# marict/nnue-vision

Measured on AMD Instinct MI355X. Metric: NNUE training images/sec (full step: fwd+bwd+clip+SGD), higher is better.
Workload: dtype f32; 1 GPU; c2: NNUE 32x32 grid 10x10x8 F=800 -> 1024/128/32 -> 10, batch 512/GPU, SGD m0.9 wd2e-4 clip1.0; global_batch=512, parallelism=dp1, launch=hipGraph, steps_per_graph=26, max_active_features=453

## Files before the change

### nnue-vision_amd/csrc/classifier_kernels.hip

```cpp
#include <type_traits>
#include <cstdlib>
#include <cstring>

#include "common.h"
#include "small_wgrad.h"

namespace {

using f32x4 = __attribute__((ext_vector_type(4))) float;

__device__ __forceinline__ float act_fn(float z, float clip) {
  const float r = z <= 0.0f ? 0.0f : z;
  return (clip > 0.0f && r > clip) ? clip : r;
}
__device__ __forceinline__ float gate_fn(float d, float h, float clip) {
  if (clip > 0.0f) return (h > 0.0f && h < clip) ? d : 0.0f;
  return h <= 0.0f ? 0.0f : d;
}

__device__ __forceinline__ float l0_at(const float* __restrict__ xr, int k, int half, int pairwise) {
  if (!pairwise) return xr[k];
  return k < half ? xr[k] * xr[k + half] : xr[k - half];
}

// ... 621 lines not shown
    }
  }
  const float b2v = (VEC && og < L3) ? b2[og] : 0.0f, b3v = (VEC && og < C) ? b3[og] : 0.0f;
  const int64_t y = labels[b];
  for (int j = tid; j < L2; j += NT) {
    float z = b1[j];
    int s = 0;
    for (; s + 8 <= ksplit; s += 8) {
      float v[8];
#pragma unroll
      for (int u = 0; u < 8; ++u) v[u] = part[((size_t)(s + u) * B + b) * L2 + j];
#pragma unroll
      for (int u = 0; u < 8; ++u) z += v[u];
    }
    for (; s < ksplit; ++s) z += part[((size_t)s * B + b) * L2 + j];
    const float h = act_fn(z, clip);
    h1s[j] = h;
    h1[(size_t)b * L2 + j] = h;
  }
  __syncthreads();
  for (int j0 = 0; j0 < L3; j0 += NT / 4) {
    const int j = j0 + og;
    float z = 0.f;
    if (j < L3) {
      const float* __restrict__ wr = w2 + (size_t)j * L2;
      if constexpr (VEC) {
        int k = 4 * part4;
        if (j0 == 0) {
#pragma unroll
          for (int i = 0; i < kPre2; ++i) {
            const int kk = 4 * (part4 + 4 * i);
            if (kk < L2) z = tail_dot4(w2v[i], *reinterpret_cast<const float4*>(h1s + kk), z);
          }
          k += 16 * kPre2;
        }
        for (; k < L2; k += 16) z = tail_dot4(*reinterpret_cast<const float4*>(wr + k), *reinterpret_cast<const float4*>(h1s + k), z);
      } else {
        for (int k = part4; k < L2; k += 4) z = fmaf(wr[k], h1s[k], z);
      }
    }
    z += __shfl_xor(z, 1);
    z += __shfl_xor(z, 2);
    if (j < L3 && part4 == 0) {
      const float h = act_fn(z + ((VEC && j0 == 0) ? b2v : b2[j]), clip);
      h2s[j] = h;
      h2[(size_t)b * L3 + j] = h;
    }
  }
  __syncthreads();
  for (int c0 = 0; c0 < C; c0 += NT / 4) {
    const int c = c0 + og;
    float z = 0.f;
    if (c < C) {
      const float* __restrict__ wr = w3 + (size_t)c * L3;
      if constexpr (VEC) {
        int k = 4 * part4;
        if (c0 == 0) {
#pragma unroll
          for (int i = 0; i < kPre3; ++i) {
            const int kk = 4 * (part4 + 4 * i);
            if (kk < L3) z = tail_dot4(w3v[i], *reinterpret_cast<const float4*>(h2s + kk), z);
          }
          k += 16 * kPre3;
        }
        for (; k < L3; k += 16) z = tail_dot4(*reinterpret_cast<const float4*>(wr + k), *reinterpret_cast<const float4*>(h2s + k), z);
      } else {
        for (int k = part4; k < L3; k += 4) z = fmaf(wr[k], h2s[k], z);
      }
    }
    z += __shfl_xor(z, 1);
    z += __shfl_xor(z, 2);
    if (c < C && part4 == 0) {
      z += (VEC && c0 == 0) ? b3v : b3[c];
      lgs[c] = z;
      logits[(size_t)b * C + c] = z;
    }
  }
  __syncthreads();
  float mx = -INFINITY, se = 0.f;
  if (C <= 64) {
    const int lane = tid & 63;
    const float v[1] = {lane < C ? lgs[lane] : -INFINITY};
    float m1[1], s1[1];
    ce_wave_stats<1>(v, lane < C, m1, s1);
    mx = m1[0];
    se = s1[0];
  } else {
    for (int c = tid; c < C; c += NT) mx = fmaxf(mx, lgs[c]);
    mx = block_reduce_nt<NT>(mx, true, red);
    for (int c = tid; c < C; c += NT) se += expf(lgs[c] - mx);
    se = block_reduce_nt<NT>(se, false, red);
  }
  const bool ok = y >= 0 && y < C;
  if (tid == 0) sample_loss[b] = ok ? nnue_ce_sample_loss(mx, lgs[y], se) : 0.0f;
  const float inv = 1.0f / se;
  __syncthreads();
  for (int c = tid; c < C; c += NT) {
    const float g = ok ? ce_dlogit(lgs[c], mx, inv, c == y, scale_over_b) : 0.0f;
    lgs[c] = g;
    d_logits[(size_t)b * C + c] = g;
  }
  __syncthreads();
  for (int j0 = 0; j0 < L3; j0 += 32) {
    const int j = j0 + (tid & 31), cp = tid >> 5;
    part_s[cp][tid & 31] = j < L3 ? dz2_slice<S>(lgs, w3 + j, cp, C, L3) : 0.0f;
    __syncthreads();
    if (cp == 0 && j < L3) {
      float q[S];
#pragma unroll
      for (int i = 0; i < S; ++i) q[i] = part_s[i][tid];
      const float v = gate_fn(slice_tree<S>(q), h2s[j], clip);
      dz2s[j] = v;
      d_z2[(size_t)b * L3 + j] = v;
    }
    __syncthreads();
  }
  for (int k = tid; k < L2; k += NT) {
    float s = 0.f;
    int j = 0;
    for (; j + 16 <= L3; j += 16) {
      float w[16];
#pragma unroll
      for (int u = 0; u < 16; ++u) w[u] = w2[(size_t)(j + u) * L2 + k];
#pragma unroll
      for (int u = 0; u < 16; ++u) s = fmaf(dz2s[j + u], w[u], s);
    }
    for (; j < L3; ++j) s = fmaf(dz2s[j], w2[(size_t)j * L2 + k], s);
    const float v = gate_fn(s, h1s[k], clip);
    d_z1[(size_t)b * L2 + k] = v;
    if (d_z1_g) d_z1_g[(size_t)g * L2 + k] = v;
  }
  __syncthreads();
}

constexpr int kTdxRows = 16, kTdxThreads = 512, kTdxMaxC = 64;

#ifdef NNUE_ABLATIONS
constexpr int kTdxClocks = 10;
struct TdxAbl { long long* clocks; };
#define NNUE_TDX_ABL_PARAM , TdxAbl abl
#define NNUE_TDX_CLOCK(i) do { if (abl.clocks && threadIdx.x == 0) abl.clocks[(size_t)blockIdx.x * kTdxClocks + (i)] = clock64(); } while (0)
#else
#define NNUE_TDX_ABL_PARAM
#define NNUE_TDX_CLOCK(i) do { } while (0)
#endif

struct TailFrags {
  float w2f[8];
  float w2b[8];
  float w3f[8];
  float b3v;
};

template <int L2, int L3>
__device__ __forceinline__ void tail_load_frags(TailFrags& f, const float* __restrict__ w2, const float* __restrict__ w3,
                                                const float* __restrict__ b3, int C, int wave, int r, int q) {
  static_assert(L2 == 128 && L3 == 32, "tail_load_frags: the wave roles are laid out for 128 / 32");
  const int t = wave & 1, kq = wave >> 1, kh = (wave >> 1) & 1;
  const bool lg = wave < 4;
#pragma unroll
  for (int i = 0; i < 8; ++i) {
    const int k = 16 * (i >> 2) + 4 * q + (i & 3);
    f.w2f[i] = w2[(16 * t + r) * L2 + 32 * kq + k];
    f.w2b[i] = w2[k * L2 + 16 * wave + r];
    const int cls = lg ? 16 * wave + r : 32 * kh + k, unit = lg ? k : 16 * t + r;
    f.w3f[i] = w3[min(cls, C - 1) * L3 + unit];
  }
  f.b3v = b3[min(16 * (wave & 3) + r, C - 1)];
}

__device__ __forceinline__ f32x4 tail_mma4(const float4& a, float b0, float b1, float b2, float b3, f32x4 acc) {
  acc = __builtin_amdgcn_mfma_f32_16x16x4f32(a.x, b0, acc, 0, 0, 0);
  acc = __builtin_amdgcn_mfma_f32_16x16x4f32(a.y, b1, acc, 0, 0, 0);
  acc = __builtin_amdgcn_mfma_f32_16x16x4f32(a.z, b2, acc, 0, 0, 0);
  acc = __builtin_amdgcn_mfma_f32_16x16x4f32(a.w, b3, acc, 0, 0, 0);
  return acc;
}

template <int L2, int L3, bool DX, bool SKIP = false>
__global__ __launch_bounds__(kTdxThreads) void tail_dx_train_kernel(
    const float* __restrict__ part, int ksplit, const float* __restrict__ b1, const float* __restrict__ w2,
    const float* __restrict__ b2, const float* __restrict__ w3, const float* __restrict__ b3, float clip,
    const int64_t* __restrict__ labels, float scale_over_b, int B, int C, float* __restrict__ h1, float* __restrict__ h2,
    float* __restrict__ logits, float* __restrict__ sample_loss, float* __restrict__ d_logits, float* __restrict__ d_z1,
    float* __restrict__ d_z2, const float* __restrict__ x, const float* __restrict__ w1, int L1, float* __restrict__ d_x,
    int m_tiles, int n_cg NNUE_TDX_ABL_PARAM) {
  constexpr int T = kTdxRows, NT = kTdxThreads, NWAVE = NT / 64;
  constexpr int NI = T * L2 / 4 / NT;
  constexpr int NCH = L2 / (16 * kBwxKC);
  static_assert(NI >= 1 && NI * NT * 4 == T * L2 && T * L3 == NT && NWAVE == 8 && T == 16,
                "tail_dx_train_kernel: unsupported layer widths");
  __shared__ __attribute__((aligned(16))) float h1s[T][L2 + 4];
  __shared__ __attribute__((aligned(16))) float dz1s[T][L2 + 4];
  __shared__ __attribute__((aligned(16))) float h2s[T][L3 + 4];
  __shared__ __attribute__((aligned(16))) float dz2s[T][L3 + 4];
  __shared__ float ps[T][4][L3];
  __shared__ __attribute__((aligned(16))) float lgs[T][kTdxMaxC + 4];
  __shared__ int64_t ys[T];
  __shared__ f32x4 xch[DX ? NWAVE : 1][64];

  const int blk = blockIdx.x, slot = blk >> 3;
  const int mt = (slot / n_cg) * 8 + (blk & 7), cg = slot % n_cg;
  if (mt >= m_tiles) return;
  const bool writer = cg == 0;
  const int row0 = mt * T;
  const int tid = threadIdx.x;
  constexpr bool skip = SKIP;
  NNUE_TDX_CLOCK(0);

  const int wave = __builtin_amdgcn_readfirstlane(tid >> 6);
  const int lane = tid & 63;
  const int r = lane & 15, q = lane >> 4;
  const int half = L1 / 2;
  const int hi = wave & 1;
  const int c0 = (cg * (NWAVE / 2) + (wave >> 1)) * 16, c1 = c0 + half, cm = hi ? c1 : c0;
  int orows[4];
#pragma unroll
  for (int e = 0; e < 4; ++e) orows[e] = row0 + 4 * q + e;
  float bw[NCH][kBwxKC][4];
  float xv[4];
  if constexpr (DX) {
#pragma unroll
    for (int n = 0; n < NCH; ++n) bwx_load_b_tile(bw[n], w1, n * 16 * kBwxKC, L1, L2, cm, r, q);
#pragma unroll
    for (int e = 0; e < 4; ++e) xv[e] = x[(size_t)min(orows[e], B - 1) * L1 + (hi ? c0 : c1) + r];
  }

  TailFrags fr;
  tail_load_frags<L2, L3>(fr, w2, w3, b3, C, wave, r, q);
  const float b2v = b2[tid % L3];
  const int64_t yv = labels[min(row0 + (tid % T), B - 1)];
  int srow[NI], scol[NI];
  float4 z4[NI];
  const float* prow[NI];
#pragma unroll
  for (int i = 0; i < NI; ++i) {
    const int f = tid + NT * i;
    srow[i] = f / (L2 / 4);
    scol[i] = 4 * (f % (L2 / 4));
    prow[i] = part + (size_t)min(row0 + srow[i], B - 1) * L2 + scol[i];
    z4[i] = make_float4(b1[scol[i]], b1[scol[i] + 1], b1[scol[i] + 2], b1[scol[i] + 3]);
  }
  const size_t slab = (size_t)B * L2;
  auto load_batch = [&](int s0, float4 (&v)[NI][16]) {
#pragma unroll
    for (int i = 0; i < NI; ++i)
#pragma unroll
      for (int u = 0; u < 16; ++u) v[i][u] = *reinterpret_cast<const float4*>(prow[i] + (size_t)min(s0 + u, ksplit - 1) * slab);
  };
  auto sum_batch = [&](int s0, const float4 (&v)[NI][16]) {
#pragma unroll
    for (int i = 0; i < NI; ++i)
#pragma unroll
      for (int u = 0; u < 16; ++u) {
        const bool add = s0 + u < ksplit;
        z4[i].x = add ? z4[i].x + v[i][u].x : z4[i].x;
        z4[i].y = add ? z4[i].y + v[i][u].y : z4[i].y;
        z4[i].z = add ? z4[i].z + v[i][u].z : z4[i].z;
        z4[i].w = add ? z4[i].w + v[i][u].w : z4[i].w;
      }
  };
  {
    float4 v[NI][16];
    load_batch(0, v);
    if (tid < T) ys[tid] = row0 + tid < B ? yv : -1;
    sum_batch(0, v);
  }
  for (int s0 = 16; s0 < ksplit; s0 += 16) {
    float4 v[NI][16];
    load_batch(s0, v);
    sum_batch(s0, v);
  }

#pragma unroll
  for (int i = 0; i < NI; ++i) {
    float4 h;
    h.x = act_fn(z4[i].x, clip); h.y = act_fn(z4[i].y, clip); h.z = act_fn(z4[i].z, clip); h.w = act_fn(z4[i].w, clip);
    *reinterpret_cast<float4*>(&h1s[srow[i]][scol[i]]) = h;
    if (writer && row0 + srow[i] < B) *reinterpret_cast<float4*>(h1 + (size_t)(row0 + srow[i]) * L2 + scol[i]) = h;
  }
  __syncthreads();
  NNUE_TDX_CLOCK(1);

  const f32x4 zero4 = (f32x4){0.f, 0.f, 0.f, 0.f};
  const int orow_t = tid / L3, ounit = tid % L3;
  {
    const int t = wave & 1, kq = wave >> 1;
    f32x4 acc = zero4;
    if constexpr (!skip) {
#pragma unroll
      for (int g = 0; g < 2; ++g) {
        const float4 a = *reinterpret_cast<const float4*>(&h1s[r][32 * kq + 16 * g + 4 * q]);
        acc = tail_mma4(a, fr.w2f[4 * g], fr.w2f[4 * g + 1], fr.w2f[4 * g + 2], fr.w2f[4 * g + 3], acc);
      }
    }
#pragma unroll
    for (int e = 0; e < 4; ++e) ps[4 * q + e][kq][16 * t + r] = acc[e];
  }
  __syncthreads();
  NNUE_TDX_CLOCK(2);
  {
    float z = ps[orow_t][0][ounit];
    z += ps[orow_t][1][ounit];
    z += ps[orow_t][2][ounit];
    z += ps[orow_t][3][ounit];
    const float h = act_fn(z + b2v, clip);
    h2s[orow_t][ounit] = h;
    if (writer && row0 + orow_t < B) h2[(size_t)(row0 + orow_t) * L3 + ounit] = h;
  }
  __syncthreads();
  NNUE_TDX_CLOCK(3);
  if (16 * wave < C) {
    const int n = 16 * wave + r;
    const bool n_in = n < C;
    f32x4 acc = zero4;
    if constexpr (!skip) {
#pragma unroll
      for (int g = 0; g < 2; ++g) {
        const float4 a = *reinterpret_cast<const float4*>(&h2s[r][16 * g + 4 * q]);
        acc = tail_mma4(a, n_in ? fr.w3f[4 * g] : 0.f, n_in ? fr.w3f[4 * g + 1] : 0.f, n_in ? fr.w3f[4 * g + 2] : 0.f,
                        n_in ? fr.w3f[4 * g + 3] : 0.f, acc);
      }
    }
    if (n_in) {
#pragma unroll
      for (int e = 0; e < 4; ++e) {
        const int rr = 4 * q + e;
        const float z = acc[e] + fr.b3v;
        lgs[rr][n] = z;
        if (writer && row0 + rr < B) logits[(size_t)(row0 + rr) * C + n] = z;
      }
    }
  }
  __syncthreads();
  NNUE_TDX_CLOCK(4);
  {
    constexpr int RW = T / NWAVE;
    const bool in = lane < C;
    float v[RW], mx[RW], se[RW];
#pragma unroll
    for (int it = 0; it < RW; ++it) v[it] = in ? lgs[wave + NWAVE * it][lane] : -INFINITY;
    ce_wave_stats_fast<RW>(v, in, mx, se);
#pragma unroll
    for (int it = 0; it < RW; ++it) {
      const int rr = wave + NWAVE * it;
      const int64_t y = ys[rr];
      const bool ok = y >= 0 && y < C;
      const float zy = ok ? lgs[rr][y] : 0.f;
      if (writer && lane == 0 && row0 + rr < B) sample_loss[row0 + rr] = ok ? nnue_ce_sample_loss(mx[it], zy, se[it]) : 0.0f;
      const float inv = 1.0f / se[it];
      if (in) {
        const float g = ok ? ce_dlogit(v[it], mx[it], inv, lane == y, scale_over_b) : 0.0f;
        lgs[rr][lane] = g;
        if (writer && row0 + rr < B) d_logits[(size_t)(row0 + rr) * C + lane] = g;
      }
    }
  }
  __syncthreads();
  NNUE_TDX_CLOCK(5);
  if (wave >= 4) {
    const int t = wave & 1, kh = (wave >> 1) & 1;
    f32x4 acc = zero4;
    if constexpr (!skip) {
#pragma unroll
      for (int g = 0; g < 2; ++g) {
        const int cb = 32 * kh + 16 * g;
        if (cb < C) {
          const int c = cb + 4 * q;
          float4 a = *reinterpret_cast<const float4*>(&lgs[r][c]);
          a.x = c < C ? a.x : 0.f; a.y = c + 1 < C ? a.y : 0.f; a.z = c + 2 < C ? a.z : 0.f; a.w = c + 3 < C ? a.w : 0.f;
          acc = tail_mma4(a, c < C ? fr.w3f[4 * g] : 0.f, c + 1 < C ? fr.w3f[4 * g + 1] : 0.f, c + 2 < C ? fr.w3f[4 * g + 2] : 0.f,
                          c + 3 < C ? fr.w3f[4 * g + 3] : 0.f, acc);
        }
      }
    }
#pragma unroll
    for (int e = 0; e < 4; ++e) ps[4 * q + e][kh][16 * t + r] = acc[e];
  }
  __syncthreads();
  NNUE_TDX_CLOCK(6);
  {
    const float s = ps[orow_t][0][ounit] + ps[orow_t][1][ounit];
    const float v = gate_fn(s, h2s[orow_t][ounit], clip);
    dz2s[orow_t][ounit] = v;
    if (writer && row0 + orow_t < B) d_z2[(size_t)(row0 + orow_t) * L3 + ounit] = v;
  }
  __syncthreads();
  NNUE_TDX_CLOCK(7);
  {
    f32x4 acc = zero4;
    if constexpr (!skip) {
#pragma unroll
      for (int g = 0; g < 2; ++g) {
        const float4 a = *reinterpret_cast<const float4*>(&dz2s[r][16 * g + 4 * q]);
        acc = tail_mma4(a, fr.w2b[4 * g], fr.w2b[4 * g + 1], fr.w2b[4 * g + 2], fr.w2b[4 * g + 3], acc);
      }
    }
    const int k = 16 * wave + r;
#pragma unroll
    for (int e = 0; e < 4; ++e) {
      const int rr = 4 * q + e;
      const float v = gate_fn(acc[e], h1s[rr][k], clip);
      dz1s[rr][k] = v;
      if (writer && row0 + rr < B) d_z1[(size_t)(row0 + rr) * L2 + k] = v;
    }
  }
  __syncthreads();
  NNUE_TDX_CLOCK(8);
  if constexpr (DX) {
    const bool row_ok = row0 + r < B;
    f32x4 acc = (f32x4){0.f, 0.f, 0.f, 0.f};
#pragma unroll
    for (int n = 0; n < NCH; ++n) {
      BwxChunk ch;
      bwx_load_a(ch, &dz1s[r][0], row_ok, n * 16 * kBwxKC, L2, q);
      bwx_mma_tile(ch.a, bw[n], acc);
    }
    xch[wave][lane] = acc;
    __syncthreads();
    const f32x4 other = xch[wave ^ 1][lane];
#pragma unroll
    for (int e = 0; e < 4; ++e) {
      const int orow = orows[e];
      if (orow >= B) continue;
      float* __restrict__ o = d_x + (size_t)orow * L1;
      if (hi) o[c1 + r] = other[e] * xv[e];
      else o[c0 + r] = fmaf(acc[e], xv[e], other[e]);
    }
  }
  NNUE_TDX_CLOCK(9);
}

struct ClsPlan {
  bool fwd_mfma, bww_mfma, bwx_mfma;
  int fwd_ksplit;
  int bww_ksplit, bww_klen;
};

int bucket_tiles(int B, int K) { return (B + 15) / 16 + K; }

bool tail_dx_supported(int B, int L1, int L2, int L3, int C, int K, int pairwise) {
  return B > 0 && K == 1 && pairwise && L1 > 0 && L1 % 128 == 0 && C >= 1 && C <= kTdxMaxC && L2 == 128 && L3 == 32;
}

ClsPlan make_plan(int B, int L1, int L2, int pairwise, int K = 1) {
  ClsPlan p{};
  p.fwd_mfma = (L1 % 32 == 0) && (L2 % 16 == 0);
  p.fwd_ksplit = 1;
  if (p.fwd_mfma) {
    const int tiles = (K > 1 ? bucket_tiles(B, K) : (B + 15) / 16) * ((L2 + 63) / 64);
    int ks = 1;
    while (tiles * ks < 1024 && L1 % (ks * 2 * 16) == 0 && L1 / (ks * 2) >= 64) ks *= 2;
    if (pairwise && ks == 1) ks = 2;
    static const int force_ks = [] { const char* e = getenv("NNUE_CLS_FWD_KSPLIT"); return e ? atoi(e) : 0; }();
    if (force_ks >= 2 && (force_ks & (force_ks - 1)) == 0 && L1 % (force_ks * 16) == 0 && L1 / force_ks >= 32) ks = force_ks;
    p.fwd_ksplit = ks;
  }
  p.bww_mfma = (L1 % 64 == 0) && (L2 % 32 == 0);
  p.bww_ksplit = 1;
  p.bww_klen = B;
  if (p.bww_mfma && K > 1) {
    const int tiles = (L2 / 32) * (L1 / 64);
    int ks = 1;
    while (tiles * ks < 512 && B / (ks * 2) >= 64) ks *= 2;
    p.bww_ksplit = ks;
    p.bww_klen = (((B + ks - 1) / ks) + 15) / 16 * 16;
  } else if (p.bww_mfma) {
    const int tiles = (L2 / 32) * (L1 / 64);
    int ks = 1;
    while (tiles * ks < 1024 && B / (ks * 2) >= 32) ks *= 2;
    p.bww_ksplit = ks;
    p.bww_klen = ((B + ks - 1) / ks + 3) / 4 * 4;
  }
  p.bwx_mfma = (L1 % 32 == 0) && (L2 % 16 == 0);
  return p;
}

int64_t plan_scratch_floats(const ClsPlan& p, int B, int L1, int L2, int L3, int K = 1) {
  const int64_t fwd = (int64_t)p.fwd_ksplit * B * L2;
  const int64_t bwd = (int64_t)B * L2 + (int64_t)B * L3 + (p.bww_ksplit > 1 ? (int64_t)p.bww_ksplit * K * L2 * L1 : 0);
  return (fwd > bwd ? fwd : bwd) + 64;
}

#include "bucket_group.h"

constexpr int kGroupThreads = 1024;
__global__ __launch_bounds__(kGroupThreads) void bucket_group_kernel(GroupArgs ga) {
  __shared__ int lds[kGroupLdsInts];
  bucket_group_body<kGroupThreads>(ga, lds);
}

Buckets no_buckets() { return Buckets{1, nullptr, nullptr, nullptr, nullptr, 0}; }

int buckets_from(const nnue_buckets* c, int B, Buckets* out, const char* who) {
  *out = no_buckets();
  if (!c || c->K <= 1) return NNUE_OK;
  NNUE_REQUIRE(c->K <= kMaxBuckets, NNUE_E_SHAPE, "%s: %d layer stacks (at most %d)", who, c->K, kMaxBuckets);
  NNUE_REQUIRE(c->bucket && c->rows && c->tile_bucket && c->seg, NNUE_E_ARG, "%s: null bucket pointer", who);
  NNUE_REQUIRE(c->tiles == bucket_tiles(B, c->K), NNUE_E_SHAPE, "%s: bucket grouping was made for another batch (tiles %d, expected %d)", who,
               c->tiles, bucket_tiles(B, c->K));
  *out = Buckets{c->K, c->bucket, c->rows, c->tile_bucket, c->seg, c->tiles};
  return NNUE_OK;
}

}

namespace {

int forward_impl(const float* x, int pairwise, const float* w1, const float* b1, const float* w2, const float* b2, const float* w3,
                 const float* b3, float clip, int B, int L1, int L2, int L3, int C, float* h1, float* h2, float* logits, void* scratch,
                 int64_t scratch_bytes, const Buckets& bk, nnue_stream_t stream) {
  NNUE_REQUIRE(x && w1 && b1 && w2 && b2 && w3 && b3 && h1 && h2 && logits && scratch, NNUE_E_ARG,
// ... 94 lines not shown

extern "C" int nnue_bucket_group(const int32_t* n, int B, int P, int K, int32_t* bucket, int32_t* rows, int32_t* tile_bucket,
                                 int32_t* seg, nnue_stream_t stream) {
  NNUE_REQUIRE(n && bucket && rows && tile_bucket && seg, NNUE_E_ARG, "nnue_bucket_group: null pointer");
  NNUE_REQUIRE(B > 0 && P >= 0 && K >= 1, NNUE_E_ARG, "nnue_bucket_group: B=%d P=%d K=%d out of range", B, P, K);
  NNUE_REQUIRE(K <= kMaxBuckets, NNUE_E_SHAPE, "nnue_bucket_group: %d layer stacks (at most %d)", K, kMaxBuckets);
  hipLaunchKernelGGL(bucket_group_kernel, dim3(1), dim3(kGroupThreads), 0, static_cast<hipStream_t>(stream),
                     GroupArgs{n, B, P, K, bucket, rows, tile_bucket, seg, bucket_tiles(B, K)});
  return nnue_launch_status("nnue_bucket_group");
}

extern "C" int nnue_classifier_forward(const float* x, int pairwise, const float* w1, const float* b1, const float* w2,
                                       const float* b2, const float* w3, const float* b3, float clip, int B, int L1,
                                       int L2, int L3, int C, float* h1, float* h2, float* logits, void* scratch,
                                       int64_t scratch_bytes, nnue_stream_t stream) {
  return forward_impl(x, pairwise, w1, b1, w2, b2, w3, b3, clip, B, L1, L2, L3, C, h1, h2, logits, scratch, scratch_bytes, no_buckets(),
                      stream);
}

extern "C" int nnue_classifier_forward_bucketed(const float* x, int pairwise, const float* w1, const float* b1, const float* w2,
                                                const float* b2, const float* w3, const float* b3, float clip, int B, int L1, int L2,
                                                int L3, int C, float* h1, float* h2, float* logits, void* scratch,
                                                int64_t scratch_bytes, const nnue_buckets* buckets, nnue_stream_t stream) {
  Buckets bk;
  const int rc = buckets_from(buckets, B, &bk, "nnue_classifier_forward_bucketed");
  if (rc != NNUE_OK) return rc;
  return forward_impl(x, pairwise, w1, b1, w2, b2, w3, b3, clip, B, L1, L2, L3, C, h1, h2, logits, scratch, scratch_bytes, bk, stream);
}

extern "C" int nnue_classifier_backward(const float* x, int pairwise, const float* w1, const float* w2, const float* w3,
                                        float clip, const float* h1, const float* h2, const float* d_logits, int B, int L1,
                                        int L2, int L3, int C, float* d_x, float* d_w1, float* d_b1, float* d_w2,
                                        float* d_b2, float* d_w3, float* d_b3, void* scratch, int64_t scratch_bytes,
                                        nnue_stream_t stream) {
  return backward_impl(x, pairwise, w1, w2, w3, clip, h1, h2, d_logits, B, L1, L2, L3, C, d_x, d_w1, d_b1, d_w2, d_b2, d_w3, d_b3, scratch,
                       scratch_bytes, no_buckets(), stream);
}

extern "C" int nnue_classifier_backward_bucketed(const float* x, int pairwise, const float* w1, const float* w2, const float* w3,
                                                 float clip, const float* h1, const float* h2, const float* d_logits, int B, int L1,
                                                 int L2, int L3, int C, float* d_x, float* d_w1, float* d_b1, float* d_w2, float* d_b2,
                                                 float* d_w3, float* d_b3, void* scratch, int64_t scratch_bytes,
                                                 const nnue_buckets* buckets, nnue_stream_t stream) {
  Buckets bk;
  const int rc = buckets_from(buckets, B, &bk, "nnue_classifier_backward_bucketed");
  if (rc != NNUE_OK) return rc;
  return backward_impl(x, pairwise, w1, w2, w3, clip, h1, h2, d_logits, B, L1, L2, L3, C, d_x, d_w1, d_b1, d_w2, d_b2, d_w3, d_b3, scratch,
                       scratch_bytes, bk, stream);
}

__global__ __launch_bounds__(256) void l1_backward_x_small_wgrad(const float* __restrict__ x, int pairwise, const float* __restrict__ w1,
                                                                 const float* __restrict__ d_z1, int B, int L1, int L2,
                                                                 float* __restrict__ d_x, int x_blocks, SmallWgrad a) {
  if ((int)blockIdx.x < x_blocks) l1_backward_x_body(x, pairwise, w1, d_z1, B, L1, L2, d_x, blockIdx.x, a.bk);
  else {
    __shared__ float red[1024];
    small_wgrad_body(a, (int)blockIdx.x - x_blocks, red);
  }
}

namespace {
struct TrainLayout {
  int64_t part, d_z1, d_z2, d_logits, slabs, d_z1_g, x_g, total;
};
TrainLayout train_layout(const ClsPlan& p, int B, int L1, int L2, int L3, int C, int K = 1) {
  TrainLayout t{};
  int64_t off = 0;
  auto take = [&](int64_t n) { const int64_t o = off; off += nnue_round_up(n, 4); return o; };
  const int64_t ext = (L1 % 64 == 0) ? L1 / 64 : 0;
  t.part = take((p.fwd_ksplit > ext ? (int64_t)p.fwd_ksplit : ext) * B * L2);
  t.d_z1 = take((int64_t)B * L2);
  t.d_z2 = take((int64_t)B * L3);
  t.d_logits = take((int64_t)B * C);
  t.slabs = take(p.bww_ksplit > 1 ? (int64_t)p.bww_ksplit * K * L2 * L1 : 0);
  const int64_t grows = K > 1 ? (int64_t)bucket_tiles(B, K) * 16 : 0;
  t.d_z1_g = take(grows * L2);
  t.x_g = take(grows * L1);
  t.total = off + 4;
  return t;
}

#ifdef NNUE_ABLATIONS
long long* g_tdx_clocks = nullptr;
int g_tdx_clock_blocks = 0;
#endif

int train_step_impl(const float* x, int pairwise, const float* w1, const float* b1, const float* w2, const float* b2, const float* w3,
                    const float* b3, float clip, const int64_t* labels, float grad_scale, int B, int L1, int L2, int L3, int C, float* h1,
                    float* h2, float* logits, float* sample_loss, float* loss, float* d_x, float* d_w1, float* d_b1, float* d_w2,
                    float* d_b2, float* d_w3, float* d_b3, void* scratch, int64_t scratch_bytes, int phases, const Buckets& bk,
                    nnue_stream_t stream) {
  NNUE_REQUIRE(x && w1 && b1 && w2 && b2 && w3 && b3 && labels && h1 && h2 && logits && sample_loss && loss && scratch,
               NNUE_E_ARG, "nnue_classifier_train_step: null pointer");
  const bool fuse_tail = phases == 123;
  if (fuse_tail) phases = 59;
  NNUE_REQUIRE(phases >= 1 && phases <= 63 && (phases & 3) && (phases & 20) != 20 && (!(phases & 32) || (phases & 19) == 19), NNUE_E_ARG,
               "nnue_classifier_train_step: phases = 1 (activations + d_x) | 2 (weight gradients + loss) [| 4: first-layer weight product beside "
               "d_x] [| 8: layer-1 slabs already at the start of scratch] [| 16 (not with 4): d_w1 comes from nnue_ftm_backward] [| 32 (with 1, 2 "
               "and 16): the small gradients and the mean loss ride in nnue_ftm_backward's launch as well] [| 64 (only as 123 = 59 + 64): the "
               "per-sample tail runs in the d_x launch]");
  const bool ext_dw1 = (phases & 16) != 0;
  const bool ext_small = (phases & 32) != 0;
  const bool ext_slabs = (phases & 8) != 0;
  const int K = bk.K;
  NNUE_REQUIRE(K == 1 || !ext_slabs, NNUE_E_ARG,
               "nnue_classifier_train_step: phases bit 8 (layer-1 slabs formed in the FeatureTransformer forward's epilogue) exists for one layer stack only");
  NNUE_REQUIRE(K == 1 || !ext_dw1 || (pairwise && L1 % 4 == 0), NNUE_E_SHAPE,
               "nnue_classifier_train_step: phases bit 16 with K > 1 needs the pairwise block and L1 %% 4 == 0");
  NNUE_REQUIRE(!ext_slabs || (pairwise && L1 % 64 == 0), NNUE_E_SHAPE,
               "nnue_classifier_train_step: phases bit 8 needs the pairwise block and L1 %% 64 == 0 (got L1=%d)", L1);
  NNUE_REQUIRE(d_w1 && d_b1 && d_w2 && d_b2 && d_w3 && d_b3, NNUE_E_ARG, "nnue_classifier_train_step: null gradient pointer");
  NNUE_REQUIRE(B > 0 && L1 > 0 && L2 > 0 && L3 > 0 && C > 0, NNUE_E_ARG,
               "nnue_classifier_train_step: B=%d L1=%d L2=%d L3=%d C=%d must be positive", B, L1, L2, L3, C);
  NNUE_REQUIRE(!pairwise || L1 % 2 == 0, NNUE_E_SHAPE, "nnue_classifier_train_step: pairwise needs an even L1 (got %d)", L1);
  const int64_t tail_lds = ((int64_t)L2 + 2 * L3 + C + 8) * 4;
  NNUE_REQUIRE(tail_lds <= 64 * 1024, NNUE_E_SHAPE, "nnue_classifier_train_step: L2+2*L3+C too large for the LDS tail");
  const ClsPlan p = make_plan(B, L1, L2, pairwise, K);
  const TrainLayout t = train_layout(p, B, L1, L2, L3, C, K);
  NNUE_REQUIRE(scratch_bytes >= t.total * (int64_t)sizeof(float), NNUE_E_SCRATCH,
               "nnue_classifier_train_step: scratch %lld < %lld bytes", (long long)scratch_bytes, (long long)(t.total * 4));
  NNUE_REQUIRE(nnue_aligned16(x) && nnue_aligned16(w1) && nnue_aligned16(scratch) && nnue_aligned16(d_w1) && nnue_aligned16(h1) &&
                   nnue_aligned16(h2),
               NNUE_E_ARG, "nnue_classifier_train_step: pointers must be 16-byte aligned");
  hipStream_t s = static_cast<hipStream_t>(stream);
  float* base = static_cast<float*>(scratch);
  float *part = base + t.part, *d_z1 = base + t.d_z1, *d_z2 = base + t.d_z2, *d_logits = base + t.d_logits, *slabs = base + t.slabs;
  const bool grouped = K > 1 && ext_dw1;
  float* d_z1_g = grouped ? base + t.d_z1_g : nullptr;
  float* x_g = grouped ? base + t.x_g : nullptr;
  const int tail_grid = grouped ? bk.tiles * 16 : B;
  const bool slab_pass = p.bww_mfma && p.bww_ksplit > 1;
  const int m_tiles = bk.rows ? bk.tiles : (B + 15) / 16;
  const bool early_bww = (phases & 4) && p.bwx_mfma && p.bww_mfma && d_x != nullptr;
  const int tail_slabs = ext_slabs ? L1 / 64 : p.fwd_ksplit;
  const int wgrad_blocks = small_wgrad_tiles(L2, L3, C) * K + 1;
  const long long count = (long long)K * L2 * L1;
  const int slab_blocks = slab_pass && !ext_dw1 ? (int)((count / 4 + 255) / 256) : 0;
  const SmallWgrad sw{d_logits, d_z2, d_z1, h1, h2, B, L2, L3, C, d_w3, d_b3, d_w2, d_b2, d_b1, sample_loss, loss, wgrad_blocks,
                      slabs, slab_pass && !ext_dw1 ? p.bww_ksplit : 0, count, d_w1, bk, p.bww_klen};
  const bool wgrad_rides = (phases & 3) == 3 && ext_dw1 && p.bwx_mfma && d_x != nullptr;
  NNUE_REQUIRE(!ext_small || wgrad_rides, NNUE_E_SHAPE,
               "nnue_classifier_train_step: phases bit 32 needs the d_x launch the small gradients otherwise ride in (MFMA shapes, d_x requested)");
  NNUE_REQUIRE(!fuse_tail || tail_dx_supported(B, L1, L2, L3, C, K, pairwise), NNUE_E_SHAPE,
               "nnue_classifier_train_step: phases 123 (tail inside the d_x launch) needs nnue_classifier_train_fused_tail_supported "
               "(B=%d L1=%d L2=%d L3=%d C=%d K=%d pairwise=%d)", B, L1, L2, L3, C, K, pairwise);
  NNUE_REQUIRE(!fuse_tail || (nnue_aligned16(w2) && nnue_aligned16(w3)), NNUE_E_ARG,
               "nnue_classifier_train_step: phases 123 needs 16-byte aligned w2 and w3");
  const bool tile_tail = tail_dx_supported(B, L1, L2, L3, C, K, pairwise);
  auto launch_tile_tail = [&](bool dx, int slabs_in) {
    const int n_cg = dx ? L1 / 32 / (kTdxThreads / 128) : 1;
    const int tdx_grid = (m_tiles + 7) / 8 * 8 * n_cg;
#ifdef NNUE_ABLATIONS
    static const int abl_skip = [] { const char* e = getenv("NNUE_CLS_ABL_SKIP_TAIL_PRODUCTS"); return e ? atoi(e) : 0; }();
    static const int abl_clocks = [] { const char* e = getenv("NNUE_CLS_ABL_TAIL_CLOCKS"); return e ? atoi(e) : 0; }();
    if (abl_clocks && tdx_grid > g_tdx_clock_blocks) {
      if (g_tdx_clocks) (void)hipFree(g_tdx_clocks);
      g_tdx_clocks = nullptr;
      g_tdx_clock_blocks = hipMalloc(&g_tdx_clocks, (size_t)tdx_grid * kTdxClocks * sizeof(long long)) == hipSuccess ? tdx_grid : 0;
    }
    if (abl_clocks && g_tdx_clocks) (void)hipMemsetAsync(g_tdx_clocks, 0, (size_t)g_tdx_clock_blocks * kTdxClocks * sizeof(long long), s);
    const TdxAbl abl{abl_clocks ? g_tdx_clocks : nullptr};
#define NNUE_TDX_ABL_ARG , abl
#else
    constexpr int abl_skip = 0;
#define NNUE_TDX_ABL_ARG
#endif
#define NNUE_TDX(DX, SKIP)                                                                                                                \
  hipLaunchKernelGGL((tail_dx_train_kernel<128, 32, DX, SKIP>), dim3(tdx_grid), dim3(kTdxThreads), 0, s, part, slabs_in, b1, w2, b2, w3, b3, \
                     clip, labels, grad_scale / (float)B, B, C, h1, h2, logits, sample_loss, d_logits, d_z1, d_z2, x, w1, L1, d_x, m_tiles, \
                     n_cg NNUE_TDX_ABL_ARG)
    if (abl_skip) {
#ifdef NNUE_ABLATIONS
      if (dx) NNUE_TDX(true, true); else NNUE_TDX(false, true);
#endif
    } else if (dx) NNUE_TDX(true, false);
    else NNUE_TDX(false, false);
#undef NNUE_TDX
#undef NNUE_TDX_ABL_ARG
  };
  if (fuse_tail) {
    launch_tile_tail(true, L1 / 64);
    return nnue_launch_status("nnue_classifier_train_step");
  }
  if (phases & 1) {
    if (ext_slabs) {
    } else if (p.fwd_mfma) {
      const long long waves = (long long)m_tiles * ((L2 + 63) / 64) * p.fwd_ksplit;
      hipLaunchKernelGGL(l1_forward_mfma, dim3((unsigned)((waves + 3) / 4)), dim3(256), 0, s, x, pairwise, w1, B, L1, L2, p.fwd_ksplit, part, bk);
    } else {
      const long long waves = (long long)B * L2;
      hipLaunchKernelGGL(l1_forward_simple, dim3((unsigned)((waves + 3) / 4)), dim3(256), 0, s, x, pairwise, w1, B, L1, L2, part, bk);
    }
    const bool vec = L2 % 4 == 0 && L3 % 4 == 0 && nnue_aligned16(w2) && nnue_aligned16(w3);
#define NNUE_TAIL(NT, V)                                                                                                                  \
  hipLaunchKernelGGL((tail_train_kernel<NT, V>), dim3(tail_grid), dim3(NT), (size_t)tail_lds, s, part, tail_slabs, b1, w2, b2, w3, b3, clip, \
                     labels, grad_scale / (float)B, B, L2, L3, C, h1, h2, logits, sample_loss, d_logits, d_z1, d_z2, bk, x, L1, x_g, d_z1_g)
    if (tile_tail) launch_tile_tail(false, tail_slabs);
    else if (C > 256) { if (vec) NNUE_TAIL(512, true); else NNUE_TAIL(512, false); }
    else { if (vec) NNUE_TAIL(128, true); else NNUE_TAIL(128, false); }
#undef NNUE_TAIL
    if (d_x) {
      if (p.bwx_mfma && early_bww) {
        const long long xw = (long long)m_tiles * (L1 / 32), ww = (long long)K * (L2 / 32) * (L1 / 64) * p.bww_ksplit;
        const int w_blocks = (int)((ww + 3) / 4);
        hipLaunchKernelGGL(l1_backward_xw_mfma, dim3((unsigned)(w_blocks + (xw + 3) / 4)), dim3(256), 0, s, x, pairwise, w1, d_z1, B, L1, L2,
                           d_x, w_blocks, p.bww_ksplit, p.bww_klen, slab_pass ? slabs : d_w1, bk);
      } else if (wgrad_rides) {
        const long long waves = (long long)m_tiles * (L1 / 32);
        const int x_blocks = (int)((waves + 3) / 4);
#ifdef NNUE_ABLATIONS
        static const int skip_small = [] { const char* e = getenv("NNUE_CLS_ABL_SKIP_SMALL"); return e ? atoi(e) : 0; }();
#else
        constexpr int skip_small = 0;
#endif
        hipLaunchKernelGGL(l1_backward_x_small_wgrad, dim3((unsigned)(x_blocks + ((skip_small || ext_small) ? 0 : wgrad_blocks))), dim3(256), 0, s, x, pairwise, w1,
                           (const float*)d_z1, B, L1, L2, d_x, x_blocks, sw);
      } else if (p.bwx_mfma) {
        const long long waves = (long long)m_tiles * (L1 / 32);
        hipLaunchKernelGGL(l1_backward_x_mfma, dim3((unsigned)((waves + 3) / 4)), dim3(256), 0, s, x, pairwise, w1, d_z1, B, L1, L2, d_x, bk);
      } else {
        const int cols = pairwise ? L1 / 2 : L1;
        hipLaunchKernelGGL(l1_backward_x_simple, dim3(B, (cols + 255) / 256), dim3(256), 0, s, x, pairwise, w1, d_z1, B, L1, L2, d_x, bk);
      }
    }
  }
  if (wgrad_rides) return nnue_launch_status("nnue_classifier_train_step");
  if (phases & 2) {
    if (early_bww || ext_dw1) {
    } else if (p.bww_mfma) {
      const long long waves = (long long)K * (L2 / 32) * (L1 / 64) * p.bww_ksplit;
      hipLaunchKernelGGL(l1_backward_w_mfma, dim3((unsigned)((waves + 3) / 4)), dim3(256), 0, s, x, pairwise, d_z1, B, L1, L2, p.bww_ksplit,
                         p.bww_klen, slab_pass ? slabs : d_w1, bk);
    } else {
      hipLaunchKernelGGL(l1_backward_w_simple, dim3(K * L2, (L1 + 255) / 256), dim3(256), 0, s, x, pairwise, d_z1, B, L1, L2, d_w1, bk);
    }
    hipLaunchKernelGGL(small_wgrad_kernel, dim3(wgrad_blocks + slab_blocks), dim3(256), 0, s, sw);
  }
  return nnue_launch_status("nnue_classifier_train_step");
}
}

#ifdef NNUE_ABLATIONS
extern "C" int nnue_cls_abl_tail_clocks(long long* out, int max_blocks) {
  if (!g_tdx_clocks || !out) return -1;
  const int n = g_tdx_clock_blocks < max_blocks ? g_tdx_clock_blocks : max_blocks;
  if (hipDeviceSynchronize() != hipSuccess) return -1;
  if (hipMemcpy(out, g_tdx_clocks, (size_t)n * kTdxClocks * sizeof(long long), hipMemcpyDeviceToHost) != hipSuccess) return -1;
  return n;
}
#endif

extern "C" int64_t nnue_classifier_train_scratch(int B, int L1, int L2, int L3, int C) {
  return nnue_classifier_train_scratch_bucketed(B, L1, L2, L3, C, 1);
}

extern "C" int64_t nnue_classifier_train_scratch_bucketed(int B, int L1, int L2, int L3, int C, int K) {
  if (B <= 0 || L1 <= 0 || L2 <= 0 || L3 <= 0 || C <= 0 || K <= 0) return 0;
  const int64_t a = train_layout(make_plan(B, L1, L2, 0, K), B, L1, L2, L3, C, K).total;
  const int64_t b = train_layout(make_plan(B, L1, L2, 1, K), B, L1, L2, L3, C, K).total;
  return (a > b ? a : b) * (int64_t)sizeof(float);
}

extern "C" int nnue_classifier_train_fused_tail_supported(int B, int L1, int L2, int L3, int C, int K, int pairwise) {
  return tail_dx_supported(B, L1, L2, L3, C, K, pairwise) ? 1 : 0;
}

extern "C" int64_t nnue_classifier_train_dz1_offset(int B, int L1, int L2, int L3, int C, int pairwise) {
  if (B <= 0 || L1 <= 0 || L2 <= 0 || L3 <= 0 || C <= 0) return -1;
  return train_layout(make_plan(B, L1, L2, pairwise), B, L1, L2, L3, C).d_z1 * (int64_t)sizeof(float);
}

extern "C" int64_t nnue_classifier_train_dz1_grouped_offset(int B, int L1, int L2, int L3, int C, int K) {
  if (B <= 0 || L1 <= 0 || L2 <= 0 || L3 <= 0 || C <= 0 || K <= 1 || K > kMaxBuckets) return -1;
  return train_layout(make_plan(B, L1, L2, 1, K), B, L1, L2, L3, C, K).d_z1_g * (int64_t)sizeof(float);
}

extern "C" int64_t nnue_classifier_train_x_grouped_offset(int B, int L1, int L2, int L3, int C, int K) {
  if (B <= 0 || L1 <= 0 || L2 <= 0 || L3 <= 0 || C <= 0 || K <= 1 || K > kMaxBuckets) return -1;
  return train_layout(make_plan(B, L1, L2, 1, K), B, L1, L2, L3, C, K).x_g * (int64_t)sizeof(float);
}

extern "C" int nnue_classifier_train_rider(int pairwise, int B, int L1, int L2, int L3, int C, const float* h1, const float* h2,
                                           const float* sample_loss, float* loss, float* d_b1, float* d_w2, float* d_b2, float* d_w3,
                                           float* d_b3, void* scratch, int64_t scratch_bytes, const nnue_buckets* buckets,
                                           nnue_cls_rider* out) {
  NNUE_REQUIRE(h1 && h2 && sample_loss && loss && d_b1 && d_w2 && d_b2 && d_w3 && d_b3 && scratch && out, NNUE_E_ARG,
               "nnue_classifier_train_rider: null pointer");
  NNUE_REQUIRE(B > 0 && L1 > 0 && L2 > 0 && L3 > 0 && C > 0, NNUE_E_ARG, "nnue_classifier_train_rider: sizes must be positive");
  Buckets bk;
  const int rc = buckets_from(buckets, B, &bk, "nnue_classifier_train_rider");
  if (rc != NNUE_OK) return rc;
  const ClsPlan p = make_plan(B, L1, L2, pairwise, bk.K);
  const TrainLayout t = train_layout(p, B, L1, L2, L3, C, bk.K);
  NNUE_REQUIRE(scratch_bytes >= t.total * (int64_t)sizeof(float), NNUE_E_SCRATCH, "nnue_classifier_train_rider: scratch %lld < %lld bytes",
               (long long)scratch_bytes, (long long)(t.total * 4));
  float* base = static_cast<float*>(scratch);
  const int wgrad_blocks = small_wgrad_tiles(L2, L3, C) * bk.K + 1;
  const SmallWgrad sw{base + t.d_logits, base + t.d_z2, base + t.d_z1, h1, h2, B, L2, L3, C, d_w3, d_b3, d_w2, d_b2, d_b1, sample_loss, loss,
                      wgrad_blocks, nullptr, 0, (long long)bk.K * L2 * L1, nullptr, bk, p.bww_klen};
  static_assert(sizeof(SmallWgrad) <= sizeof(nnue_cls_rider), "nnue_cls_rider is too small");
  memset(out, 0, sizeof(*out));
  memcpy(out, &sw, sizeof(sw));
  return NNUE_OK;
}

extern "C" int nnue_classifier_train_step(const float* x, int pairwise, const float* w1, const float* b1, const float* w2,
                                          const float* b2, const float* w3, const float* b3, float clip,
                                          const int64_t* labels, float grad_scale, int B, int L1, int L2, int L3, int C,
                                          float* h1, float* h2, float* logits, float* sample_loss, float* loss, float* d_x,
                                          float* d_w1, float* d_b1, float* d_w2, float* d_b2, float* d_w3, float* d_b3,
                                          void* scratch, int64_t scratch_bytes, int phases, nnue_stream_t stream) {
  return train_step_impl(x, pairwise, w1, b1, w2, b2, w3, b3, clip, labels, grad_scale, B, L1, L2, L3, C, h1, h2, logits, sample_loss, loss,
                         d_x, d_w1, d_b1, d_w2, d_b2, d_w3, d_b3, scratch, scratch_bytes, phases, no_buckets(), stream);
}

extern "C" int nnue_classifier_train_step_bucketed(const float* x, int pairwise, const float* w1, const float* b1, const float* w2,
                                                   const float* b2, const float* w3, const float* b3, float clip, const int64_t* labels,
                                                   float grad_scale, int B, int L1, int L2, int L3, int C, float* h1, float* h2,
                                                   float* logits, float* sample_loss, float* loss, float* d_x, float* d_w1, float* d_b1,
                                                   float* d_w2, float* d_b2, float* d_w3, float* d_b3, void* scratch,
                                                   int64_t scratch_bytes, int phases, const nnue_buckets* buckets, nnue_stream_t stream) {
  Buckets bk;
  const int rc = buckets_from(buckets, B, &bk, "nnue_classifier_train_step_bucketed");
  if (rc != NNUE_OK) return rc;
  return train_step_impl(x, pairwise, w1, b1, w2, b2, w3, b3, clip, labels, grad_scale, B, L1, L2, L3, C, h1, h2, logits, sample_loss, loss,
                         d_x, d_w1, d_b1, d_w2, d_b2, d_w3, d_b3, scratch, scratch_bytes, phases, bk, stream);
}
```

Baseline: 8.326 million images/sec.

## Defer tail kernel operand loads to just before each phase that uses them

```diff
diff --git a/nnue-vision_amd/csrc/classifier_kernels.hip b/nnue-vision_amd/csrc/classifier_kernels.hip
--- a/nnue-vision_amd/csrc/classifier_kernels.hip
+++ b/nnue-vision_amd/csrc/classifier_kernels.hip
@@ -797,21 +797,43 @@
   float b3v;
 };
 
-template <int L2, int L3>
-__device__ __forceinline__ void tail_load_frags(TailFrags& f, const float* __restrict__ w2, const float* __restrict__ w3,
-                                                const float* __restrict__ b3, int C, int wave, int r, int q) {
-  static_assert(L2 == 128 && L3 == 32, "tail_load_frags: the wave roles are laid out for 128 / 32");
-  const int t = wave & 1, kq = wave >> 1, kh = (wave >> 1) & 1;
-  const bool lg = wave < 4;
-#pragma unroll
-  for (int i = 0; i < 8; ++i) {
-    const int k = 16 * (i >> 2) + 4 * q + (i & 3);
-    f.w2f[i] = w2[(16 * t + r) * L2 + 32 * kq + k];
-    f.w2b[i] = w2[k * L2 + 16 * wave + r];
-    const int cls = lg ? 16 * wave + r : 32 * kh + k, unit = lg ? k : 16 * t + r;
-    f.w3f[i] = w3[min(cls, C - 1) * L3 + unit];
-  }
-  f.b3v = b3[min(16 * (wave & 3) + r, C - 1)];
+template <bool VEC>
+__device__ __forceinline__ void tail_load4(float* __restrict__ out, const float* __restrict__ p) {
+  if constexpr (VEC) {
+    const f32x4 v = *reinterpret_cast<const f32x4*>(p);
+#pragma unroll
+    for (int e = 0; e < 4; ++e) out[e] = v[e];
+  } else {
+#pragma unroll
+    for (int e = 0; e < 4; ++e) out[e] = p[e];
+  }
+}
+
+template <int L2, bool VEC>
+__device__ __forceinline__ void tail_load_frag_h2(TailFrags& f, const float* __restrict__ w2, int wave, int r, int q) {
+  const int t = wave & 1, kq = wave >> 1;
+#pragma unroll
+  for (int g = 0; g < 2; ++g) tail_load4<VEC>(&f.w2f[4 * g], w2 + (16 * t + r) * L2 + 32 * kq + 16 * g + 4 * q);
+}
+
+template <int L3, bool VEC>
+__device__ __forceinline__ void tail_load_frag_logits(TailFrags& f, const float* __restrict__ w3, int C, int wave, int r, int q) {
+  const int cls = min(16 * wave + r, C - 1);
+#pragma unroll
+  for (int g = 0; g < 2; ++g) tail_load4<VEC>(&f.w3f[4 * g], w3 + cls * L3 + 16 * g + 4 * q);
+}
+
+template <int L3>
+__device__ __forceinline__ void tail_load_frag_dz2(TailFrags& f, const float* __restrict__ w3, int C, int wave, int r, int q) {
+  const int t = wave & 1, kh = (wave >> 1) & 1;
+#pragma unroll
+  for (int i = 0; i < 8; ++i) f.w3f[i] = w3[min(32 * kh + 16 * (i >> 2) + 4 * q + (i & 3), C - 1) * L3 + 16 * t + r];
+}
+
+template <int L2>
+__device__ __forceinline__ void tail_load_frag_dz1(TailFrags& f, const float* __restrict__ w2, int wave, int r, int q) {
+#pragma unroll
+  for (int i = 0; i < 8; ++i) f.w2b[i] = w2[(16 * (i >> 2) + 4 * q + (i & 3)) * L2 + 16 * wave + r];
 }
 
 __device__ __forceinline__ f32x4 tail_mma4(const float4& a, float b0, float b1, float b2, float b3, f32x4 acc) {
@@ -822,7 +844,7 @@
   return acc;
 }
 
-template <int L2, int L3, bool DX, bool SKIP = false>
+template <int L2, int L3, bool DX, bool SKIP = false, bool NOLOAD = false>
 __global__ __launch_bounds__(kTdxThreads) void tail_dx_train_kernel(
     const float* __restrict__ part, int ksplit, const float* __restrict__ b1, const float* __restrict__ w2,
     const float* __restrict__ b2, const float* __restrict__ w3, const float* __restrict__ b3, float clip,
@@ -833,7 +855,7 @@
   constexpr int T = kTdxRows, NT = kTdxThreads, NWAVE = NT / 64;
   constexpr int NI = T * L2 / 4 / NT;
   constexpr int NCH = L2 / (16 * kBwxKC);
-  static_assert(NI >= 1 && NI * NT * 4 == T * L2 && T * L3 == NT && NWAVE == 8 && T == 16,
+  static_assert(L2 == 128 && L3 == 32 && NI >= 1 && NI * NT * 4 == T * L2 && T * L3 == NT && NWAVE == 8 && T == 16,
                 "tail_dx_train_kernel: unsupported layer widths");
   __shared__ __attribute__((aligned(16))) float h1s[T][L2 + 4];
   __shared__ __attribute__((aligned(16))) float dz1s[T][L2 + 4];
@@ -856,24 +878,6 @@
   const int wave = __builtin_amdgcn_readfirstlane(tid >> 6);
   const int lane = tid & 63;
   const int r = lane & 15, q = lane >> 4;
-  const int half = L1 / 2;
-  const int hi = wave & 1;
-  const int c0 = (cg * (NWAVE / 2) + (wave >> 1)) * 16, c1 = c0 + half, cm = hi ? c1 : c0;
-  int orows[4];
-#pragma unroll
-  for (int e = 0; e < 4; ++e) orows[e] = row0 + 4 * q + e;
-  float bw[NCH][kBwxKC][4];
-  float xv[4];
-  if constexpr (DX) {
-#pragma unroll
-    for (int n = 0; n < NCH; ++n) bwx_load_b_tile(bw[n], w1, n * 16 * kBwxKC, L1, L2, cm, r, q);
-#pragma unroll
-    for (int e = 0; e < 4; ++e) xv[e] = x[(size_t)min(orows[e], B - 1) * L1 + (hi ? c0 : c1) + r];
-  }
-
-  TailFrags fr;
-  tail_load_frags<L2, L3>(fr, w2, w3, b3, C, wave, r, q);
-  const float b2v = b2[tid % L3];
   const int64_t yv = labels[min(row0 + (tid % T), B - 1)];
   int srow[NI], scol[NI];
   float4 z4[NI];
@@ -886,6 +890,7 @@
     prow[i] = part + (size_t)min(row0 + srow[i], B - 1) * L2 + scol[i];
     z4[i] = make_float4(b1[scol[i]], b1[scol[i] + 1], b1[scol[i] + 2], b1[scol[i] + 3]);
   }
+  __builtin_amdgcn_sched_barrier(0);
   const size_t slab = (size_t)B * L2;
   auto load_batch = [&](int s0, float4 (&v)[NI][16]) {
 #pragma unroll
@@ -905,17 +910,31 @@
         z4[i].w = add ? z4[i].w + v[i][u].w : z4[i].w;
       }
   };
-  {
-    float4 v[NI][16];
-    load_batch(0, v);
-    if (tid < T) ys[tid] = row0 + tid < B ? yv : -1;
-    sum_batch(0, v);
-  }
+  float4 v0[NI][16];
+  load_batch(0, v0);
+  __builtin_amdgcn_sched_barrier(0);
+
+  TailFrags fr;
+  if constexpr (NOLOAD) {
+#pragma unroll
+    for (int i = 0; i < 8; ++i) fr.w2f[i] = fr.w2b[i] = fr.w3f[i] = 0.5f;
+    fr.b3v = 0.5f;
+  } else {
+    tail_load_frag_h2<L2, DX>(fr, w2, wave, r, q);
+    fr.b3v = b3[min(16 * (wave & 3) + r, C - 1)];
+  }
+  const float b2v = b2[tid % L3];
+  __builtin_amdgcn_sched_barrier(0);
+
+
+  ys[tid % T] = row0 + (tid % T) < B ? yv : -1;
+  sum_batch(0, v0);
   for (int s0 = 16; s0 < ksplit; s0 += 16) {
     float4 v[NI][16];
     load_batch(s0, v);
     sum_batch(s0, v);
   }
+
 
 #pragma unroll
   for (int i = 0; i < NI; ++i) {
@@ -926,6 +945,50 @@
   }
   __syncthreads();
   NNUE_TDX_CLOCK(1);
+  __builtin_amdgcn_sched_barrier(0);
+  if constexpr (!NOLOAD) tail_load_frag_logits<L3, DX>(fr, w3, C, wave & 3, r, q);
+  __builtin_amdgcn_sched_barrier(0);
+
+  const int half = L1 / 2;
+  const int hi = wave & 1;
+  const int c0 = (cg * (NWAVE / 2) + (wave >> 1)) * 16, c1 = c0 + half, cm = hi ? c1 : c0;
+  int orows[4];
+#pragma unroll
+  for (int e = 0; e < 4; ++e) orows[e] = row0 + 4 * q + e;
+  float bw[NCH][kBwxKC][4];
+  float xv[4];
+  if constexpr (DX && NOLOAD) {
+#pragma unroll
+    for (int n = 0; n < NCH; ++n)
+#pragma unroll
+      for (int u = 0; u < kBwxKC; ++u)
+#pragma unroll
+        for (int e = 0; e < 4; ++e) bw[n][u][e] = 0.5f;
+#pragma unroll
+    for (int e = 0; e < 4; ++e) xv[e] = 0.5f;
+  }
+  auto load_bw = [&](int n, int u) {
+    if constexpr (DX && !NOLOAD) {
+      const float* __restrict__ wk = w1 + (size_t)(n * 16 * kBwxKC + 16 * u + 4 * q) * L1 + r;
+#pragma unroll
+      for (int e = 0; e < 4; ++e) bw[n][u][e] = wk[(size_t)e * L1 + cm];
+    }
+  };
+  auto load_xv = [&]() {
+    if constexpr (DX && !NOLOAD) {
+#pragma unroll
+      for (int e = 0; e < 4; ++e) xv[e] = x[(size_t)min(orows[e], B - 1) * L1 + (hi ? c0 : c1) + r];
+    }
+  };
+  static_assert(NCH == 2 && NCH * 16 * kBwxKC == L2, "tail_dx_train_kernel: the W1 slice is requested in two halves");
+  auto load_late = [&](bool dz2_role) {
+    if constexpr (!NOLOAD) {
+      if (dz2_role) tail_load_frag_dz2<L3>(fr, w3, C, wave, r, q);
+      tail_load_frag_dz1<L2>(fr, w2, wave, r, q);
+    }
+#pragma unroll
+    for (int u = 0; u < kBwxKC; ++u) load_bw(0, u);
+  };
 
   const f32x4 zero4 = (f32x4){0.f, 0.f, 0.f, 0.f};
   const int orow_t = tid / L3, ounit = tid % L3;
@@ -955,6 +1018,7 @@
   }
   __syncthreads();
   NNUE_TDX_CLOCK(3);
+  if (wave >= NWAVE / 2) load_late(true);
   if (16 * wave < C) {
     const int n = 16 * wave + r;
     const bool n_in = n < C;
@@ -983,11 +1047,22 @@
     constexpr int RW = T / NWAVE;
     const bool in = lane < C;
     float v[RW], mx[RW], se[RW];
+    __builtin_amdgcn_sched_barrier(0);
+    load_bw(1, 0); load_bw(1, 1);
+    __builtin_amdgcn_sched_barrier(0);
 #pragma unroll
     for (int it = 0; it < RW; ++it) v[it] = in ? lgs[wave + NWAVE * it][lane] : -INFINITY;
     ce_wave_stats_fast<RW>(v, in, mx, se);
+    __builtin_amdgcn_sched_barrier(0);
+    load_bw(1, 2); load_bw(1, 3);
+    __builtin_amdgcn_sched_barrier(0);
 #pragma unroll
     for (int it = 0; it < RW; ++it) {
+      if (it == RW - 1) {
+        __builtin_amdgcn_sched_barrier(0);
+        load_xv();
+        __builtin_amdgcn_sched_barrier(0);
+      }
       const int rr = wave + NWAVE * it;
       const int64_t y = ys[rr];
       const bool ok = y >= 0 && y < C;
@@ -1003,6 +1078,7 @@
   }
   __syncthreads();
   NNUE_TDX_CLOCK(5);
+  if (wave < NWAVE / 2) load_late(false);
   if (wave >= 4) {
     const int t = wave & 1, kh = (wave >> 1) & 1;
     f32x4 acc = zero4;
@@ -1403,6 +1479,7 @@
     const int tdx_grid = (m_tiles + 7) / 8 * 8 * n_cg;
 #ifdef NNUE_ABLATIONS
     static const int abl_skip = [] { const char* e = getenv("NNUE_CLS_ABL_SKIP_TAIL_PRODUCTS"); return e ? atoi(e) : 0; }();
+    static const int abl_noload = [] { const char* e = getenv("NNUE_CLS_ABL_TAIL_NO_OPERAND_LOADS"); return e ? atoi(e) : 0; }();
     static const int abl_clocks = [] { const char* e = getenv("NNUE_CLS_ABL_TAIL_CLOCKS"); return e ? atoi(e) : 0; }();
     if (abl_clocks && tdx_grid > g_tdx_clock_blocks) {
       if (g_tdx_clocks) (void)hipFree(g_tdx_clocks);
@@ -1413,19 +1490,23 @@
     const TdxAbl abl{abl_clocks ? g_tdx_clocks : nullptr};
 #define NNUE_TDX_ABL_ARG , abl
 #else
-    constexpr int abl_skip = 0;
+    constexpr int abl_skip = 0, abl_noload = 0;
 #define NNUE_TDX_ABL_ARG
 #endif
-#define NNUE_TDX(DX, SKIP)                                                                                                                \
-  hipLaunchKernelGGL((tail_dx_train_kernel<128, 32, DX, SKIP>), dim3(tdx_grid), dim3(kTdxThreads), 0, s, part, slabs_in, b1, w2, b2, w3, b3, \
-                     clip, labels, grad_scale / (float)B, B, C, h1, h2, logits, sample_loss, d_logits, d_z1, d_z2, x, w1, L1, d_x, m_tiles, \
-                     n_cg NNUE_TDX_ABL_ARG)
-    if (abl_skip) {
+#define NNUE_TDX(DX, SKIP, NOLOAD)                                                                                                        \
+  hipLaunchKernelGGL((tail_dx_train_kernel<128, 32, DX, SKIP, NOLOAD>), dim3(tdx_grid), dim3(kTdxThreads), 0, s, part, slabs_in, b1, w2, b2, \
+                     w3, b3, clip, labels, grad_scale / (float)B, B, C, h1, h2, logits, sample_loss, d_logits, d_z1, d_z2, x, w1, L1, d_x,   \
+                     m_tiles, n_cg NNUE_TDX_ABL_ARG)
+    if (abl_noload) {
 #ifdef NNUE_ABLATIONS
-      if (dx) NNUE_TDX(true, true); else NNUE_TDX(false, true);
+      if (dx) NNUE_TDX(true, false, true); else NNUE_TDX(false, false, true);
 #endif
-    } else if (dx) NNUE_TDX(true, false);
-    else NNUE_TDX(false, false);
+    } else if (abl_skip) {
+#ifdef NNUE_ABLATIONS
+      if (dx) NNUE_TDX(true, true, false); else NNUE_TDX(false, true, false);
+#endif
+    } else if (dx) NNUE_TDX(true, false, false);
+    else NNUE_TDX(false, false, false);
 #undef NNUE_TDX
 #undef NNUE_TDX_ABL_ARG
   };
```

Result: faster. 8.424 million images/sec, median of 6 (+1.2%).
